# lhoangan/arap_flow

Hardware: AMD Instinct MI355X
Metric: ARAP solve+warp frames/sec at 854x480 mesh (higher is better)
Workload: dtype f32; 1 GPU; configs[1]: single 854x480 DAVIS-shaped frame, single-segment mask, fd=1; schedule 19/8/400; segments_per_frame=1, fd=1, parallelism=frames sharded, no collective, grid_vertices_per_frame=409920

## Files before the change

### arap_flow_amd/capi.py

```python
import ctypes as C
import os

_HERE = os.path.dirname(os.path.abspath(__file__))
LIB_PATH = os.environ.get("ARAPOPT_LIB") or os.path.join(_HERE, "lib", "libarapopt.so")


class Opt_InitializationParameters(C.Structure):
    _fields_ = [("doublePrecision", C.c_int), ("verbosityLevel", C.c_int),
                ("collectPerKernelTimingInfo", C.c_int), ("threadsPerBlock", C.c_int)]


class MeshStats(C.Structure):
    _fields_ = [("vertices", C.c_uint32), ("outside", C.c_uint32), ("triangles", C.c_uint32), ("folded", C.c_uint32),
                ("nonfinite", C.c_uint32), ("reserved", C.c_uint32), ("det_min", C.c_float), ("det_max", C.c_float),
                ("disp2_max", C.c_float)]


MESH_STATS_KEYS = tuple(k for k, _ in MeshStats._fields_ if k != "reserved")


_VP, _U, _I = C.c_void_p, C.c_uint, C.c_int
SYMBOLS = [
    ("Opt_NewState", _VP, [Opt_InitializationParameters]),
    ("Opt_ProblemDefine", _VP, [_VP, C.c_char_p, C.c_char_p]),
# ... 22 lines not shown
    ("ArapFlow_SolverSolve", _I, [_VP, _U, _U, _U, _U]),
    ("ArapFlow_SolverSolveAsync", _I, [_VP, _U, _U, _U, _U, _I, _I]),
    ("ArapFlow_SolverWait", _I, [_VP]),
    ("ArapFlow_SolverHostResults", _I, [_VP, _U, C.POINTER(_VP), C.POINTER(_VP), C.POINTER(_VP)]),
    ("ArapFlow_SolverWarp", _I, [_VP, _U]),
    ("ArapFlow_SolverGetResults", _I, [_VP, _U, _VP, _VP, _VP, _VP, _VP, C.POINTER(C.c_double)]),
    ("ArapFlow_SolverStats", _I, [_VP, C.POINTER(C.c_uint64), C.POINTER(C.c_uint64), C.POINTER(C.c_uint64)]),
    ("ArapFlow_SetResident", None, [_VP, _I]),
    ("ArapFlow_SetTile", _I, [_VP, _I, _I]),
    ("ArapFlow_SolverResidentLaunches", C.c_uint64, [_VP]),
    ("ArapFlow_PlanResidentLaunches", C.c_uint64, [_VP]),
    ("ArapFlow_SolverLaunchesFor", _I, [_VP, C.c_uint]),
    ("ArapFlow_ResidentDeal", _I, [C.POINTER(C.c_int), C.c_uint, C.POINTER(C.c_int), C.c_uint]),
    ("ArapFlow_ResidentTiles", _I, [_VP, _U, _U, _I, C.POINTER(C.c_int), _U, C.POINTER(C.c_int)]),
    ("ArapFlow_SolverResidentLayout", _I, [_VP, C.POINTER(C.c_int), C.POINTER(C.c_int)]),
    ("ArapFlow_SolverLeanStream", _I, [_VP]),
    ("ArapFlow_ResidentFailed", _I, [_VP]),
    ("ArapFlow_SolverStamps", _I, [_VP, _VP]),
    ("ArapFlow_SolverStampParts", _I, [_VP, _VP]),
    ("ArapFlow_WarpScratchBytes", C.c_uint64, [_U, _U]),
    ("ArapFlow_Warp", _I, [_VP, _U, _U, _VP, _VP, _VP, _VP, _VP, _VP]),
    ("ArapFlow_SolverSetOutputs", _I, [_VP, _I]),
    ("ArapFlow_SolverGetExtraResults", _I, [_VP, _U, _VP, _VP, _VP]),
    ("ArapFlow_SolverHostExtraResults", _I, [_VP, _U, C.POINTER(_VP), C.POINTER(_VP), C.POINTER(_VP)]),
    ("ArapFlow_WarpExScratchBytes", C.c_uint64, [_U, _U]),
    ("ArapFlow_WarpEx", _I, [_VP, _U, _U, _VP, _VP, _VP, _VP, _VP, _VP, _VP, _VP, _VP]),
    ("ArapFlow_SolverSetSnapshots", _I, [_VP, C.POINTER(C.c_uint), _U]),
    ("ArapFlow_SolverGetSnapshot", _I, [_VP, _U, _U, _VP, _VP, _VP, _VP]),
    ("ArapFlow_SolverHostSnapshot", _I, [_VP, _U, _U, C.POINTER(_VP), C.POINTER(_VP), C.POINTER(_VP), C.POINTER(_VP)]),
    ("ArapFlow_WarpStep", _I, [_VP, _U, _U, _VP, _VP, _VP, _VP, _VP, _VP, _VP]),
# ... 38 lines not shown
```

### arap_flow_amd/csrc/abi_solver.h

```cpp
#pragma once

namespace arap {
struct FrameExt {
    float2* bwd;
    uint8_t *occ_bwd, *occ;
    unsigned *cell, *rank;
    int4* bin;
};
struct MidDev {
    float2 *state, *flow, *step;
    uint8_t *rgb, *mask;
};
}

extern "C" int ArapFlow_SolverWait(ArapFlow_Solver* s);

enum { G_BASE, G_EXTRA, G_MID, G_DIAG, G_COUNT, MAX_PLANES = 5 };
enum { SEL_ALWAYS = 0, SEL_RGB = -1 , SEL_DEVICE = -2  };
struct Plane {
    size_t per_vertex, fixed;
    int sel;
    const void* (*dev)(const ArapFlow_Solver* s, unsigned slot, unsigned k);
};
static unsigned group_items(int g, unsigned state) { return g == G_MID ? state : state != 0; }
// ... 617 lines not shown
    build_resident_tiles(mask_red, (int)W, (int)H, aligned != 0, tiles, bx, nullptr);
    if (origins)
        for (size_t i = 0; i < tiles.size() && i < cap; ++i) origins[i] = tiles[i];
    if (bandx0)
        for (size_t i = 0; i < bx.size(); ++i) bandx0[i] = bx[i];
    return (int)tiles.size();
}
int ArapFlow_SolverResidentLayout(ArapFlow_Solver* s, int* launches_per_step, int* solves_in_flight)
{
    if (!s) return -1;
    const bool res = plan_resident_eligible(s->plan) && s->plan->res_sets > 0;
    if (launches_per_step) *launches_per_step = res ? s->plan->res_sets : 0;
    if (solves_in_flight) *solves_in_flight = res ? s->plan->res_inflight : 0;
    return 0;
}
int ArapFlow_ResidentFailed(Opt_State* state) { return state && state->resident_failed ? 1 : 0; }
int ArapFlow_SolverLeanStream(ArapFlow_Solver* s) { return s && plan_lean_stream(s->plan) ? 1 : 0; }

static int solver_stamp_table(ArapFlow_Solver* s, int table, uint64_t* out)
{
    if (!s || !s->plan->rd.stamps) return -1;
    HC(hipStreamSynchronize(s->st->stream));
    HC(hipMemcpy(out, s->plan->rd.stamps + table * RES_WGS * 16, RES_WGS * 16 * sizeof(unsigned long long), hipMemcpyDeviceToHost));
    return 0;
}
int ArapFlow_SolverStamps(ArapFlow_Solver* s, uint64_t* out) { return solver_stamp_table(s, 0, out); }
int ArapFlow_SolverStampParts(ArapFlow_Solver* s, uint64_t* out) { return solver_stamp_table(s, 1, out); }

}
```

### arap_flow_amd/csrc/arap_resident.h

```cpp
#pragma once
#include <type_traits>
#include "arap_device.h"

namespace arap {

constexpr int RES_WGS = 512;
constexpr int RES_MAX_GROUPS = 16;
constexpr int RES_THREADS = 256;
constexpr int RES_SLOTS = 9;
constexpr int RES_TILES_PER_WG = RES_SLOTS;
constexpr int RT_X = 32, RT_Y = 8;
constexpr int RES_ZX = 2 * RT_X + 2 * RT_Y;
constexpr int RES_ZG = 2 * RES_ZX;
constexpr int RES_MAX_L = 32000;
static_assert(RT_X * RT_Y == RES_THREADS && RT_Y == 2 * (RES_THREADS / 64), "one vertex per lane, two rows per wavefront");
constexpr int RES_MAX_HALO = RES_TILES_PER_WG * (2 * RT_X + 2 * RT_Y);
constexpr int RES_HALO_PER_THREAD = (RES_MAX_HALO + RES_THREADS - 1) / RES_THREADS;
constexpr int RES_MAX_TILES = RES_WGS * RES_TILES_PER_WG;
constexpr int LROW = RT_X + 2;
constexpr int LROWS = RT_Y + 2;
constexpr int LPLANE = LROW * LROWS;
constexpr int LTILE = 5 * LPLANE;
constexpr int RES_LDS_BYTES = RES_TILES_PER_WG * LTILE * 4
                              + ((RES_MAX_HALO * 8 + 15) / 16) * 16
// ... 3 lines not shown
#ifndef RES_HALO_REG_SLOTS
#define RES_HALO_REG_SLOTS 8
#endif
#ifndef RES_WREG_SLOTS
#define RES_WREG_SLOTS 7
#endif
#ifndef RES_WREG_8
#define RES_WREG_8 2
#endif
#ifndef RES_WREG_9
#define RES_WREG_9 2
#endif
#ifndef RES_WREG_FIT
#define RES_WREG_FIT 6
#endif
#ifndef RES_FIRST_LOOK
#define RES_FIRST_LOOK 5
#endif
#ifndef RES_FIRST_LOOK_2
#define RES_FIRST_LOOK_2 14
#endif
#ifndef RES_FIRST_LOOK_X
#define RES_FIRST_LOOK_X 20
#endif
#ifndef RES_OWN_LOCAL
#define RES_OWN_LOCAL 1
#endif
#ifndef RES_POLL_SLEEP
#define RES_POLL_SLEEP 1
#endif
constexpr unsigned RES_SPIN_LIMIT = 1u << 18;
#ifndef RES_GRAN_STRIDE
#define RES_GRAN_STRIDE 2
#endif
constexpr int RES_GS = RES_GRAN_STRIDE;
constexpr int RES_GRAN_UNITS = 2 * RES_WGS;
constexpr int RES_GRAN_L1 = 2 * RES_GRAN_UNITS * RES_GS;
constexpr int RES_GRAN2_STRIDE = 16;
constexpr int RES_GRAN2_GROUP = 2 * 8 * RES_GRAN2_STRIDE;
constexpr int RES_GRAN_X = RES_GRAN_L1 + 4 * RES_GRAN2_GROUP;
constexpr int RES_GRAN_PER_LAUNCH = RES_GRAN_X + RES_GRAN_L1;
#ifndef RES_FLAT_MAX_RUNS
#define RES_FLAT_MAX_RUNS 2
#endif

struct ResWg {
    int slot;
    int rank;
    int wgs;
    int gran;
};

struct ResDev {
    const int* tilelist;
    const int* ntiles;
    const int* tilepos;
    const int* bandx0;
    unsigned long long* zx;
    int rtX, rtY;
// ... 256 lines not shown
    v = wave_sum_l63_full(v);
    if (tb) { asm volatile("" :: "v"(v)); c1 = __builtin_amdgcn_s_memtime(); tb[0] += c1 - c0; c0 = c1; }
    const int wave = threadIdx.x >> 6, lane = threadIdx.x & 63;
    if (lane == 63) wsum[wave] = v;
    __syncthreads();
    double t = 0.0;
    if (wave == 0) {
        const double a = wsum[lane & 3], b = wsum[(lane & 3) ^ 1];
        if (tb) { asm volatile("s_waitcnt lgkmcnt(0)" ::: "memory"); c1 = __builtin_amdgcn_s_memtime(); tb[1] += c1 - c0; c0 = c1; }
        t = dpp_add_f64_full<0x112, 0xf>(a + b);
        if (tb) { asm volatile("" :: "v"(t)); c1 = __builtin_amdgcn_s_memtime(); tb[2] += c1 - c0; }
    }
    return t;
}

template <bool STAMPS, int NS>
__global__ __launch_bounds__(RES_THREADS, 2) void k_pcg_resident(PlanDev pd, ResDev rd, int L)
{
    static_assert(NS >= 1 && NS <= RES_SLOTS, "slots");
    unsigned long long tA = 0, tS1 = 0, tB = 0, tS2 = 0, tU = 0, t0 = 0, t1 = 0;
    unsigned long long tm[6] = {0, 0, 0, 0, 0, 0}, tbs = 0, tzr = 0;
    unsigned long long tbp[3] = {0, 0, 0}, tarr[2] = {0, 0};
#define RES_STAMP(acc) do { if (STAMPS) { t1 = __builtin_amdgcn_s_memrealtime(); acc += t1 - t0; t0 = t1; } } while (0)
    extern __shared__ __attribute__((aligned(16))) float lds[];
    const ResWg me = rd.wgmap[blockIdx.x];
    if (me.slot < 0) return;
    const int rank = me.rank;
    if (rd.force_fail) {
        if (threadIdx.x == 0) atomicExch(rd.err, 0xDEADFFFFu);
        return;
    }
    if (__hip_atomic_load(rd.err, __ATOMIC_RELAXED, __HIP_MEMORY_SCOPE_AGENT) != 0u) return;
    const int b = me.slot;
    const int wgs = me.wgs;
    const int W = pd.W, H = pd.H;
    const size_t gb = (size_t)b * pd.N;
    const int tid = threadIdx.x, lane = tid & 63, wave = tid >> 6;
    const int lx = lane & (RT_X - 1), ly = (wave << 1) | (lane >> 5);
    unsigned short* hlist = (unsigned short*)(lds + RES_TILES_PER_WG * LTILE);
    int2* tbase = (int2*)((char*)hlist + ((RES_MAX_HALO * 8 + 15) / 16) * 16);
    float* moLUT = (float*)(tbase + RES_TILES_PER_WG + 1);
    float* bcast = moLUT + 12;
    int* nhalo = (int*)(bcast + 4);
    double* wsum = (double*)(bcast + 6);
    unsigned* nbits = (unsigned*)(wsum + 10);
    unsigned* nremote = nbits + 16;
    float4* zst = (float4*)((char*)lds + RES_LDS_BYTES - RES_TILES_PER_WG * RES_ZX * 16);
    unsigned long long* gran_group = rd.gran + me.gran;
    unsigned long long* granx_group = rd.gran + RES_GRAN_X + me.gran;

    const int nt = rd.ntiles[b];
    const int tbase_n = nt / wgs, textra = nt - tbase_n * wgs;
    const int tp = tbase_n + (rank < textra ? 1 : 0);
    const int tfirst = rank * tbase_n + (rank < textra ? rank : textra);
    const int* tl = rd.tilelist + (size_t)b * RES_MAX_TILES;
    float wr2, wf2;
    {
        const Slot sl = pd.slots[b];
        wr2 = sl.wr * sl.wr;
        wf2 = sl.wf * sl.wf;
        if (tid < 10) {
            const int deg = tid % 5, fit = tid / 5;
            float dO = 0.f;
            for (int k = 0; k < deg; ++k) dO = dO + (sl.wr * sl.wr + sl.wr * sl.wr);
            if (fit) dO = fmaf(sl.wf, sl.wf, dO);
            moLUT[tid] = ginv(dO);
        }
        if (tid == 0) { *nhalo = 0; *nremote = 0u; }
        if (tid < 16) nbits[tid] = 0u;
    }

    float rx[NS], ry[NS], ra[NS];
    float dx_[NS], dy_[NS], da_[NS];
    float apx[NS], apy[NS], apa[NS];
    float ma_[NS], mo_[NS];
    unsigned fl[NS];
    int ibase[NS];
    constexpr int NWR = NS <= RES_WREG_SLOTS ? 4 : (NS == 8 ? RES_WREG_8 : RES_WREG_9);
    constexpr bool WREG = NWR > 0;
    float we[WREG ? NS : 1][5];
    const int loff = lx + W * ly;

    const int cell = (ly + 1) * LROW + (lx + 1);
#define TP2(T) ((float2*)(T))
#define TCS(T) ((float2*)(T) + LPLANE)
#define TPA(T) ((T) + 4 * LPLANE)

    int org_[NS];
#pragma unroll
    for (int j = 0; j < NS; ++j) org_[j] = j < tp ? tl[tfirst + j] : -1;
    unsigned long long* const zx_b = rd.zx + (size_t)b * RES_MAX_TILES * RES_ZG;
    for (int c = tid; c < tp * RES_ZG; c += RES_THREADS)
        __hip_atomic_store(zx_b + (size_t)tfirst * RES_ZG + c, 0ull, __ATOMIC_RELAXED, __HIP_MEMORY_SCOPE_AGENT);
// ... 55 lines not shown
        }
        fl[j] = qF[j];
        ibase[j] = __builtin_amdgcn_readfirstlane(x0 + W * y0);
        if (tid == 0) tbase[j] = make_int2(x0, y0);
    }
    float rho = read_scalar(pd.red + ((size_t)b * pd.nslots + 0) * NSHARD);
    __syncthreads();
#pragma unroll
    for (int j = 0; j < NS; ++j) {
        const unsigned f = fl[j];
        if (WREG) {
            if (NWR > 0) we[j][0] = keep_if<0>(f, wr2);
            if (NWR > 1) we[j][1] = keep_if<1>(f, wr2);
            if (NWR > 2) we[j][2] = keep_if<2>(f, wr2);
            if (NWR > 3) we[j][3] = keep_if<3>(f, wr2);
            if (NS <= RES_WREG_FIT) we[j][4] = keep_if<4>(f, wf2);
        }
        halo_append(ly == 0 && (f & F_E3), (unsigned short)(j * LPLANE + 0 * LROW + lx + 1), hlist, nhalo);
        halo_append(ly == RT_Y - 1 && (f & F_E2), (unsigned short)(j * LPLANE + (RT_Y + 1) * LROW + lx + 1), hlist, nhalo);
        halo_append(lx == 0 && (f & F_E1), (unsigned short)(j * LPLANE + (ly + 1) * LROW + 0), hlist, nhalo);
        halo_append(lx == RT_X - 1 && (f & F_E0), (unsigned short)(j * LPLANE + (ly + 1) * LROW + RT_X + 1), hlist, nhalo);
    }
    __syncthreads();
    const int nh = *nhalo;
    uint2* htab = (uint2*)hlist;
    constexpr bool HREG = NS <= RES_HALO_REG_SLOTS;
    uint2 hreg[RES_HALO_PER_THREAD];
    {
        uint2 e[RES_HALO_PER_THREAD];
#pragma unroll
        for (int u = 0; u < RES_HALO_PER_THREAD; ++u) {
// ... 36 lines not shown
            offP[n] = (unsigned)(cell + dn[n]) * 8u;
            offA[n] = (unsigned)(cell + dn[n]) * 4u;
            asm volatile("" : "+v"(offP[n]));
            asm volatile("" : "+v"(offA[n]));
        }
    }
    const int zent = border_entry(lx, ly);
    bool alive = true;
    float alpha_last = 0.f;
    asm volatile("s_waitcnt vmcnt(0)" ::: "memory");
    __syncthreads();
    bool fast = false, zfast = false;
    bool hier = false, subfast = false;
    bool hierx = false;
    unsigned long long* const gran2 =
        rd.gran + RES_GRAN_L1 + ((((int)(blockIdx.x & 7u) - (me.rank >> 6)) >> 1) & 3) * RES_GRAN2_GROUP;
    {
        const unsigned xcc = __builtin_amdgcn_s_getreg((3 << 11) | (0 << 6) | 20) & 15u;
        float dummy;
        const double mine = (double)xcc + 65536.0 * (double)(xcc * xcc);
        alive = group_sum(mine, 1u, gran_group, rank, wgs, bcast, rd.err, dummy, false, wsum + 8);
        const double tot = wsum[8];
        const double s2 = floor(tot / 65536.0), s1 = tot - 65536.0 * s2;
        fast = rd.allow_fast && ((double)wgs * s2 == s1 * s1);
        __syncthreads();
        hier = !fast && wgs > 64;
        hierx = hier && (((wgs + 63) >> 6) <= 2 || ((wgs + 63) >> 6) <= rd.flat_runs);
        if (!fast && rd.allow_fast && alive) {
            if (wave == 0) {
                const unsigned long long* buf = gran_group + (size_t)1 * wgs * RES_GS;
                bool remote = false, elsewhere = false;
                for (int m = lane; m < wgs; m += 64) {
                    const bool nb = ((nbits[(m >> 5) & 15] >> (m & 31)) & 1u) != 0u;
                    const bool same_run = hier && (m >> 6) == (rank >> 6);
                    if (nb || same_run) {
                        const unsigned long long lo = __hip_atomic_load(buf + RES_GS * m, __ATOMIC_RELAXED, __HIP_MEMORY_SCOPE_AGENT);
                        const unsigned long long hi = __hip_atomic_load(buf + RES_GS * m + 1, __ATOMIC_RELAXED, __HIP_MEMORY_SCOPE_AGENT);
                        const double val = __longlong_as_double((long long)((hi << 32) | (lo & 0xffffffffull)));
                        const double q2 = floor(val / 65536.0);
                        const bool other = (unsigned)(lo >> 32) != 1u || (unsigned)(hi >> 32) != 1u ||
                                           (unsigned)(val - 65536.0 * q2) != xcc;
                        remote = remote || (nb && other);
                        elsewhere = elsewhere || (same_run && other);
                    }
                }
                const unsigned any_remote = __any(remote) ? 1u : 0u, any_elsewhere = __any(elsewhere) ? 2u : 0u;
                if (lane == 0) *nremote = any_remote | any_elsewhere;
            }
            __syncthreads();
            zfast = (*nremote & 1u) == 0u;
            subfast = hier && (*nremote & 2u) == 0u;
        } else {
            zfast = fast;
        }
        __syncthreads();
    }
#ifndef RES_PRIO_HI
#define RES_PRIO_HI 2
#endif
#ifndef RES_PRIO_TAIL
#define RES_PRIO_TAIL 2
#endif
#define RES_PRIO(J) { if ((J) + RES_PRIO_TAIL >= NS) __builtin_amdgcn_s_setprio(0); else __builtin_amdgcn_s_setprio(RES_PRIO_HI); }
#define RES_PRIO_END() __builtin_amdgcn_s_setprio(0);
    if (STAMPS) t0 = __builtin_amdgcn_s_memrealtime();
    for (int l = 0; l < L && alive; ++l) {
// ... 52 lines not shown
                    const float2 t = fma2(make_float2(NQX, NQY), pa2, e);                              \
                    const float2 u = fma2(make_float2(NHX, NHY), make_float2(qA, qA), e + t);          \
                    axy = fma2(make_float2(w, w), u, axy);                                             \
                    aa = fmaf(-w, fmaf(QX, t.x, (QY) * t.y), aa);                                      \
                    (void)cn; (void)sn;                                                                \
                }
                RES_EDGE(0, 0,     -si,  ci,   -sn,  cn,    si, -ci)
                RES_EDGE(1, 1,      si, -ci,    sn, -cn,   -si,  ci)
                __builtin_amdgcn_sched_barrier(0);
                if (j + 1 < NS) RES_LOAD_B(j + 1)
                __builtin_amdgcn_sched_barrier(0);
                RES_EDGE(2, 2,     -ci, -si,   -cn, -sn,    ci,  si)
                RES_EDGE(3, 3,      ci,  si,    cn,  sn,   -ci, -si)
#undef RES_EDGE
                {
                    const float wf = (WREG && NS <= RES_WREG_FIT) ? we[WREG ? j : 0][4] : keep_if<4>(f, wf2);
                    axy = fma2(make_float2(wf, wf), pv, axy);
                }
                const float ax = axy.x, ay = axy.y;
                apx[j] = ax; apy[j] = ay; apa[j] = aa;
                acc += (double)dot3(pv.x, pv.y, pa_, ax, ay, aa);
            }
            __builtin_amdgcn_sched_barrier(0);
        }
#undef RES_LOAD_A
#undef RES_LOAD_B
        float sigma;
        RES_PRIO_END()
        RES_STAMP(tA);
        {
            const unsigned long long cb = STAMPS ? __builtin_amdgcn_s_memtime() : 0ull;
            const double bs = block_sum8(acc, wsum, STAMPS ? tbp : nullptr);
            if (STAMPS) tbs += __builtin_amdgcn_s_memtime() - cb;
            alive = hierx ? group_sum_x(block_sum_uniform(bs), 2u * l + 2u, gran_group, granx_group, rank, wgs, bcast, rd.err, sigma, subfast)
                  : hier  ? group_sum_h(block_sum_uniform(bs), 2u * l + 2u, gran_group, gran2, rank, wgs, bcast, rd.err, sigma, subfast)
                          : group_sum(bs, 2u * l + 2u, gran_group, rank, wgs, bcast, rd.err, sigma, fast, nullptr, rd.nowait != 0,
                                      STAMPS ? tm : nullptr, STAMPS ? tarr : nullptr);
        }
        asm volatile("" : "+v"(sigma));
        if (!alive) break;
        RES_STAMP(tS1);
        float alpha = 0.f;
        if (sigma > 0.f) alpha = rho / sigma;
        acc = 0.0;
        const unsigned ztag = 2u * l + 3u;
#pragma unroll
        for (int j = 0; j < NS; ++j) {
            RES_PRIO(j)
            unsigned f = fl[j];
            asm volatile("" : "+v"(f));
// ... 20 lines not shown
                const float2* const st2 = (const float2*)zst;
                const unsigned sh = (tid & 1) ? 16u : 0u;
                static_assert(((RES_THREADS - 64) & 1) == 0, "a thread keeps the parity of its granules");
                if (zfast) {
                    for (int g = tid - 64; g < tp * RES_ZG; g += RES_THREADS - 64) {
                        const float2 v = st2[g];
                        st_tagged(out + g, (ztag << 16) | ((__float_as_uint(v.y) >> sh) & 0xffffu), v.x, true);
                    }
                } else {
                    for (int g = tid - 64; g < tp * RES_ZG; g += RES_THREADS - 64) {
                        const float2 v = st2[g];
                        st_tagged(out + g, (ztag << 16) | ((__float_as_uint(v.y) >> sh) & 0xffffu), v.x, false);
                    }
                }
            }
            alive = hierx ? group_sum_x(block_sum_uniform(bs), 2u * l + 3u, gran_group, granx_group, rank, wgs, bcast, rd.err, rhoNew, subfast)
                  : hier  ? group_sum_h(block_sum_uniform(bs), 2u * l + 3u, gran_group, gran2, rank, wgs, bcast, rd.err, rhoNew, subfast)
                          : group_sum(bs, 2u * l + 3u, gran_group, rank, wgs, bcast, rd.err, rhoNew, fast, nullptr, rd.nowait != 0,
                                      STAMPS ? tm : nullptr, STAMPS ? tarr + 1 : nullptr);
        }
        unsigned long long hg[RES_HALO_PER_THREAD][2];
        unsigned hpk_[HREG ? 1 : RES_HALO_PER_THREAD];
#define RES_HPK(U) (HREG ? hreg[U].y : hpk_[HREG ? 0 : (U)])
#pragma unroll
        for (int u = 0; u < RES_HALO_PER_THREAD; ++u) {
            hg[u][0] = hg[u][1] = (unsigned long long)ztag << 48;
            if (tid + u * RES_THREADS < nh) {
                const unsigned gi = HREG ? hreg[u].x : htab[tid + u * RES_THREADS].x;
                const unsigned long long* q_ = (const unsigned long long*)((const char*)zx_b + (size_t)(gi * 8u));
#pragma unroll
                for (int c = 0; c < 2; ++c) hg[u][c] = __hip_atomic_load(q_ + c, __ATOMIC_RELAXED, __HIP_MEMORY_SCOPE_AGENT);
            }
// ... 163 lines not shown
```

### arap_flow_amd/csrc/host_plan.h

```cpp
#pragma once

static void hip_fatal(hipError_t e, const char* what, const char* file, int line)
{
    fprintf(stderr, "arapopt: HIP error %d (%s) in %s at %s:%d\n", (int)e, hipGetErrorString(e), what, file, line);
    exit((int)e ? (int)e : 1);
}
#define HC(call)                                                     \
    do {                                                             \
        hipError_t e_ = (call);                                      \
        if (e_ != hipSuccess) hip_fatal(e_, #call, __FILE__, __LINE__); \
    } while (0)

struct KernelTimer {
    struct Rec { std::string name; hipEvent_t a, b; };
    std::vector<Rec> recs;
    void clear()
    {
        for (auto& r : recs) { (void)hipEventDestroy(r.a); (void)hipEventDestroy(r.b); }
        recs.clear();
    }
    void report()
    {
        std::map<std::string, std::pair<int, double>> agg;
        for (auto& r : recs) {
// ... 23 lines not shown
}

struct Knobs {
    bool no_graph = false;
    int tile = -1;
    bool b8 = false;
    int stream_a = 0;
    bool no_resident = false;
    int force_res_fail = 0;
    bool no_xcd_fast = false;
    int flat_runs = RES_FLAT_MAX_RUNS;
    bool res_nowait = false;
    bool stamps = false;
    int res_groups = 0;
    int res_ns = 0;
};

static Knobs read_knobs()
{
    auto is = [](const char* name, char c) { const char* v = getenv(name); return v && v[0] == c; };
    auto num = [](const char* name, int absent) { const char* v = getenv(name); return v ? atoi(v) : absent; };
    Knobs k;
    k.no_graph = is("ARAPOPT_NO_GRAPH", '1');
    if (const char* tv = getenv("ARAPOPT_TILE")) {
        int tx = -1, ty = -1;
        if (sscanf(tv, "%dx%d", &tx, &ty) == 2) k.tile = tile_shape_index(tx, ty);
    }
    k.b8 = is("ARAPOPT_B8", '1');
    k.stream_a = num("ARAPOPT_STREAM_A", 0);
    k.no_resident = is("ARAPOPT_NO_RESIDENT", '1');
    k.force_res_fail = is("ARAPOPT_FORCE_RES_FAIL", '1') ? 1 : (is("ARAPOPT_FORCE_RES_FAIL", '2') ? 2 : 0);
    k.no_xcd_fast = is("ARAPOPT_NO_XCD_FAST", '1');
    k.flat_runs = num("ARAPOPT_FLAT_RUNS", RES_FLAT_MAX_RUNS);
    k.res_nowait = is("ARAPOPT_RES_NOWAIT", '1');
    k.stamps = is("ARAPOPT_STAMPS", '1');
    k.res_groups = std::max(0, num("ARAPOPT_RES_GROUPS", 0));
    k.res_ns = std::max(0, num("ARAPOPT_RES_NS", 0));
    return k;
}

struct Opt_State {
    int verbosity = 0;
    int timing = 0;
    int device = 0;
    hipStream_t stream = nullptr;
    hipStream_t cap = nullptr;
    hipStream_t own_stream = nullptr;
    hipEvent_t t0 = nullptr, t1 = nullptr;
    KernelTimer ktimer;
    bool use_graph = true;
    bool use_resident = true;
    bool resident_failed = false;
// ... 14 lines not shown
          q_tolerance = 1e-4f, function_tolerance = 1e-6f, trust_region_radius = 1e4f,
          radius_decrease_factor = 2.0f, min_lm_diagonal = 1e-6f, max_lm_diagonal = 1e32f;
    int nIterations = 10, lIterations = 10;
    int nIter = 0;
};

enum { GN_STEP_ALL = 0, GN_STEP_PREP = 1, GN_STEP_FUSED = 2 };
enum PhaseA { PA_NONE = 0, PA_DIRECT, PA_LDS_16x16, PA_LDS_32x8, PA_LDS_64x4, PA_LDS_32x16, PA_LDS_64x8,
              PA_MARCH, PA_MARCH2, PA_GRID };
enum PhaseB { PB_NONE = 0, PB_B, PB_B4, PB_B4_LEAN, PB_B4_R };
struct StepRecipe {
    bool resident = false;
    int part = GN_STEP_ALL;
    int L = -1, nb = 0, nsteps = 0;
    std::vector<int> res_ns;
    bool stamped = false;
    int list_blocks = 0;
    int a_kern = PA_NONE, b_kern = PB_NONE;
    dim3 a_grid{0, 0, 0}, a_block{0, 0, 0};
    int a_arg[3] = {0, 0, 0};
    int lag = -1;
};
static bool same_recipe(const StepRecipe& a, const StepRecipe& b)
{
    auto same3 = [](dim3 x, dim3 y) { return x.x == y.x && x.y == y.y && x.z == y.z; };
    return a.resident == b.resident && a.part == b.part && a.L == b.L && a.nb == b.nb && a.nsteps == b.nsteps &&
           a.res_ns == b.res_ns && a.stamped == b.stamped && a.list_blocks == b.list_blocks && a.a_kern == b.a_kern &&
           a.b_kern == b.b_kern && same3(a.a_grid, b.a_grid) && same3(a.a_block, b.a_block) &&
           std::equal(a.a_arg, a.a_arg + 3, b.a_arg) && a.lag == b.lag;
}

struct Opt_Plan {
    Opt_State* st = nullptr;
    int W = 0, H = 0, N = 0, batch = 1;
    PlanDev pd{};
    SolverParameters sp;
    std::vector<Slot> hslots;
    std::vector<Slot> uploaded;
    void* block = nullptr;
    int lcap = 0;
    int ccap = 0;
    int nb = 1;
// ... 11 lines not shown
    std::vector<std::vector<int>> h_tiles;
    std::vector<uint8_t> h_tiles_valid;
    std::vector<std::vector<int>> h_tilepos, h_bandx0;
    uint8_t* d_resact = nullptr;
    int* d_t64list = nullptr;
    int* d_t64n = nullptr;
    std::vector<std::vector<int>> h_t64;
    std::vector<int> h_t64n;
    int res_tiles_all = 0;
    bool hole_pending = false;
    ResWg* d_wgmap = nullptr;
    ResWg* pin_wgmap = nullptr;
    std::vector<ResWg> h_wgmap;
    int res_sets = 0;
    std::vector<int> res_ns;
    int knob_res_groups = 0, knob_res_ns = 0;
    int res_inflight = 0;
    unsigned res_launches = 0;
    bool opt_res_ok = false;
    bool prep_done = false;
    Slot opt_res_slot{};
    int* d_notgrid = nullptr;
    int kind = 0;
    void* lm_block = nullptr;
    float2* prevO = nullptr;
    float* prevA = nullptr;
    int lm_lcap = 0;
    float lm_radius = 0.f, lm_decrease = 0.f;
    double lm_prev_cost = 0.0;
    bool lm_done = false;

// ... 127 lines not shown
```

### arap_flow_amd/csrc/host_resident.h

```cpp
#pragma once

typedef void (*ResidentKernel)(PlanDev, ResDev, int);
template <bool STAMPS, int... NS>
static const void* resident_kernel_of(int ns, std::integer_sequence<int, NS...>)
{
    static const ResidentKernel table[] = {k_pcg_resident<STAMPS, NS + 1>...};
    return (const void*)table[ns - 1];
}
static const void* resident_kernel(bool stamps, int ns)
{
    if (ns < 1) ns = 1;
    if (ns > RES_SLOTS) ns = RES_SLOTS;
    return stamps ? resident_kernel_of<true>(ns, std::make_integer_sequence<int, RES_SLOTS>())
                  : resident_kernel_of<false>(ns, std::make_integer_sequence<int, RES_SLOTS>());
}

static void plan_enable_resident(Opt_Plan* p)
{
    Opt_State* st = p->st;
    const Knobs knobs = read_knobs();
    p->knob_res_groups = knobs.res_groups;
    p->knob_res_ns = knobs.res_ns;
    if (knobs.no_resident) return;
    hipDeviceProp_t prop;
    HC(hipGetDeviceProperties(&prop, st->device));
    if (prop.multiProcessorCount * 2 < RES_WGS) return;
    for (int ns = 1; ns <= RES_SLOTS; ++ns) {
        if (hipFuncSetAttribute(resident_kernel(false, ns), hipFuncAttributeMaxDynamicSharedMemorySize, RES_LDS_BYTES) !=
            hipSuccess) { (void)hipGetLastError(); return; }
        int occ = 0;
        if (hipOccupancyMaxActiveBlocksPerMultiprocessor(&occ, resident_kernel(false, ns), RES_THREADS, RES_LDS_BYTES) !=
                hipSuccess || occ < 2) {
            (void)hipGetLastError();
            return;
        }
    }
    const size_t B = (size_t)p->batch;
    const size_t sz_map = align_up(B * RES_WGS * sizeof(ResWg), 256);
    p->rd.rtX = (p->W + RT_X - 1) / RT_X;
    p->rd.rtY = (p->H + RT_Y - 1) / RT_Y;
    {
        const size_t nz = B * RES_MAX_TILES * RES_ZG * sizeof(unsigned long long);
        HC(hipMalloc((void**)&p->rd.zx, nz));
        HC(hipMemsetAsync(p->rd.zx, 0, nz, st->stream));
    }
    HC(hipHostMalloc((void**)&p->pin_wgmap, sz_map, hipHostMallocDefault));
    p->res_block = device_block(st, true, [&](Carver& part) {
        part(p->rd.gran, B * RES_GRAN_PER_LAUNCH * 8);
        part(p->rd.tilelist, B * RES_MAX_TILES * sizeof(int));
        part(p->rd.ntiles, B * sizeof(int));
        part(p->rd.err, sizeof(unsigned));
        part(p->d_wgmap, sz_map);
        part(p->rd.tilepos, B * p->rd.rtX * p->rd.rtY * sizeof(int));
        part(p->rd.bandx0, B * p->rd.rtY * sizeof(int));
        part(p->d_resact, (size_t)p->rd.rtX * p->rd.rtY);
    });
    p->pd.res_err = p->rd.err;
    p->rd.stamps = nullptr;
    p->rd.force_fail = knobs.force_res_fail == 1 ? 1 : 0;
    p->hole_pending = knobs.force_res_fail == 2;
    p->rd.allow_fast = knobs.no_xcd_fast ? 0 : 1;
    p->rd.flat_runs = knobs.flat_runs;
    p->rd.nowait = knobs.res_nowait ? 1 : 0;
    if (knobs.stamps) {
        for (int ns = 1; ns <= RES_SLOTS; ++ns)
            HC(hipFuncSetAttribute(resident_kernel(true, ns), hipFuncAttributeMaxDynamicSharedMemorySize, RES_LDS_BYTES));
        HC(hipMalloc(&p->rd.stamps, 2 * RES_WGS * 16 * sizeof(unsigned long long)));
        HC(hipMemset(p->rd.stamps, 0, 2 * RES_WGS * 16 * sizeof(unsigned long long)));
    }
    p->res_capable = true;
}

static void build_resident_tiles(const uint8_t* mask_red, int W, int H, bool aligned, std::vector<int>& tiles,
                                 std::vector<int>& bandx0, uint64_t* nactive)
{
    const int rtY = (H + RT_Y - 1) / RT_Y;
    tiles.clear();
    bandx0.assign(rtY, 0);
    std::vector<uint8_t> col(W);
    uint64_t na = 0;
    for (int band = 0; band < rtY; ++band) {
// ... 250 lines not shown
                    if (kind[b] == WIDE || bin_of[b] != (int)k) continue;
                    take_gran(b);
                    const int r0 = kind[b] == MEDIUM ? XW : 0;
                    for (int r = 0; r < part_w[b]; ++r, ++j)
                        map[(size_t)set * RES_WGS + (size_t)j * 8 + x] = ResWg{b, r0 + r, wgs_of[b], gran_of[b]};
                }
            }
            inflight = count > inflight ? count : inflight;
        }
    }
    if (map_out) map_out->swap(map);
    if (inflight_out) *inflight_out = inflight;
    return nsets;
}

static bool plan_resident_pack(Opt_Plan* p)
{
    std::vector<ResWg> map;
    const int nsets = resident_deal(p->h_ntiles.data(), p->nb, p->knob_res_groups, &map, &p->res_inflight);
    std::vector<int> ns(nsets, 1);
    for (size_t i = 0; i < map.size(); ++i)
        if (map[i].slot >= 0) {
            const int t = (p->h_ntiles[map[i].slot] + map[i].wgs - 1) / map[i].wgs;
            int& m = ns[i / RES_WGS];
            m = t > m ? t : m;
        }
    if (p->knob_res_ns > 0)
        for (int& m : ns) m = std::max(m, std::min(p->knob_res_ns, (int)RES_SLOTS));
    const bool same = nsets == p->res_sets && ns == p->res_ns && map.size() == p->h_wgmap.size() &&
                      memcmp(map.data(), p->h_wgmap.data(), map.size() * sizeof(ResWg)) == 0;
    if (same) return false;
    p->h_wgmap.swap(map);
    p->res_ns.swap(ns);
    p->res_sets = nsets;
    return true;
}

static void plan_upload_wgmap(Opt_Plan* p)
{
    Opt_State* st = p->st;
    if (p->hole_pending) {
        std::vector<ResWg> holed = p->h_wgmap;
        for (ResWg& w : holed)
            if (w.slot >= 0 && w.wgs > 1 && w.rank == w.wgs - 1) { w = ResWg{-1, 0, 0, 0}; break; }
        HC(hipStreamSynchronize(st->stream));
        HC(hipMemcpy(p->d_wgmap, holed.data(), holed.size() * sizeof(ResWg), hipMemcpyHostToDevice));
        p->hole_pending = false;
    } else {
// ... 34 lines not shown
```

### arap_flow_amd/csrc/host_step.h

```cpp
#pragma once

static bool plan_active_tiles_majority(const Opt_Plan* p)
{
    long act = 0;
    for (int b = 0; b < p->nb; ++b) act += p->h_ntiles[b];
    const long all = (long)((p->W + RT_X - 1) / RT_X) * ((p->H + RT_Y - 1) / RT_Y);
    return 2 * act >= (long)p->nb * all;
}

static bool plan_lean_stream(const Opt_Plan* p)
{
    return p->res_frames_any && p->grid_u && !p->pd.lm && p->st->tile < 0 && (p->N & 3) == 0 && !p->st->force_b8 &&
           p->st->stream_a == 0 && plan_active_tiles_majority(p);
}

static int plan_list_blocks(const Opt_Plan* p)
{
    int maxn = 1;
    for (int k = 0; k < p->nb; ++k) maxn = std::max(maxn, p->h_t64n[k]);
    return std::min((maxn + 63) / 64 * 64, p->pd.tilesX * p->pd.tilesY);
}

constexpr int MARCH_ROWS = 5, MARCH2_ROWS = 7;

static StepRecipe plan_step_recipe(Opt_Plan* p, int nsteps)
{
    const Opt_State* st = p->st;
    StepRecipe r;
    r.resident = plan_resident_eligible(p);
    r.L = p->sp.lIterations;
    r.nb = p->nb;
    r.nsteps = nsteps;
    if (r.resident) {
        if (plan_resident_pack(p)) plan_upload_wgmap(p);
        r.res_ns = p->res_ns;
        r.stamped = p->rd.stamps != nullptr;
        if (p->res_frames && st->verbosity == 0) r.part = GN_STEP_FUSED;
        if (p->res_frames && p->d_t64list != nullptr) r.list_blocks = plan_list_blocks(p);
        return r;
    }
    const bool lean = plan_lean_stream(p);
    int v = st->tile;
    if (v < 0 && p->grid_u && !p->pd.lm) {
        if (st->stream_a == 1) {
            constexpr int TX = 64, TY = 8;
            const int tX = (p->W + TX - 1) / TX, tY = (p->H + TY - 1) / TY, ch = (tX * tY + 7) / 8;
            r.a_kern = PA_GRID;
            r.a_grid = dim3((unsigned)(p->nb * 8 * ch));
            r.a_block = dim3(TX, TY, 1);
            r.a_arg[0] = tX; r.a_arg[1] = tY; r.a_arg[2] = ch;
// ... 70 lines not shown
    if (r.list_blocks > 0) {
        pd.t64list = pdl.t64list = p->d_t64list;
        pd.t64n = pdl.t64n = p->d_t64n;
        gl = dim3((unsigned)r.list_blocks, 1, (unsigned)r.nb);
    }
    if (part != GN_STEP_FUSED) LAUNCH(p, s, "GNPrep", k_gn_prep, gl, b, 0, pd);
    if (part == GN_STEP_PREP) return;
    if (part == GN_STEP_FUSED) LAUNCH(p, s, "PCGInit1", k_gn_init_resf, gl, b, 0, pd);
    else LAUNCH(p, s, "PCGInit1", k_gn_init, gl, b, 0, pdl);
    if (r.resident) {
        ResDev rd = p->rd;
        rd.fuse_update = part == GN_STEP_FUSED ? 1 : 0;
        for (size_t set = 0; set < r.res_ns.size(); ++set) {
            rd.wgmap = p->d_wgmap + set * RES_WGS;
            rd.gran = p->rd.gran + gran_per_launch * set;
            const ResidentKernel kern = (ResidentKernel)resident_kernel(r.stamped, r.res_ns[set]);
            if (r.stamped)
                hipLaunchKernelGGL(kern, dim3(RES_WGS), dim3(RES_THREADS), RES_LDS_BYTES, s, p->pd, rd, L);
            else
                LAUNCH(p, s, "PCGResident", kern, dim3(RES_WGS), dim3(RES_THREADS), RES_LDS_BYTES, p->pd, rd, L);
        }
    } else {
        for (int l = 0; l < L; ++l) {
            launch_pcg_a(p, s, r, l);
            launch_pcg_b(p, s, r, l);
        }
    }
    if (part != GN_STEP_FUSED) LAUNCH(p, s, "PCGLinearUpdate", k_gn_update, gl, b, 0, pdl, r.lag);
}

static void plan_gn_step(Opt_Plan* p, int nsteps = 1)
// ... 88 lines not shown
```

### arap_flow_amd/opt.py

```python
import ctypes as C
import math

import numpy as np
import torch

from . import capi

BUILTIN_PLAN = b"builtin:arap"


def _dev_ptr(t):
    assert t.is_cuda and t.is_contiguous()
    return C.c_void_p(t.data_ptr())


def _host_ptr(a):
    return a.ctypes.data_as(C.c_void_p) if a is not None else None


def _view(ptr, ctype, shape):
    if not ptr.value:
        return None
    return np.ctypeslib.as_array(C.cast(ptr, C.POINTER(ctype)), shape=(int(np.prod(shape)),)).reshape(shape)

# ... 374 lines not shown
            obwd = np.empty((H, W), np.uint8) if self.outputs & capi.OUT_BACKWARD else None
            occ = np.empty((H, W), np.uint8) if self.outputs & capi.OUT_OCCLUSION else None
            if self.lib.ArapFlow_SolverGetExtraResults(self.h, slot, p(bwd), p(obwd), p(occ)) != 0:
                return out
            if bwd is not None:
                out.update(backward_flow=bwd, occlusion_bwd=obwd)
            if occ is not None:
                out.update(occlusion=occ)
        return out

    def stats(self):
        a, b, c = C.c_uint64(), C.c_uint64(), C.c_uint64()
        self.lib.ArapFlow_SolverStats(self.h, C.byref(a), C.byref(b), C.byref(c))
        ls, fl = C.c_int(0), C.c_int(0)
        self.lib.ArapFlow_SolverResidentLayout(self.h, C.byref(ls), C.byref(fl))
        return dict(pcg_iterations_per_frame=a.value, active_vertices=b.value, grid_vertices=c.value,
                    resident_launches=int(self.lib.ArapFlow_SolverResidentLaunches(self.h)),
                    resident_launches_per_step=ls.value, resident_solves_in_flight=fl.value,
                    lean_stream=bool(self.lib.ArapFlow_SolverLeanStream(self.h)))

    def close(self):
        if self.h:
            self.lib.ArapFlow_SolverFree(self.h)
            self.h = None


def _warp_call(state, name, dims, inputs, outputs, scratch=None, bad_args=True, lead=()):
    lib = state.lib
    up = lambda a, dt: None if a is None else torch.from_numpy(np.ascontiguousarray(a, dt)).cuda()
    new = lambda shape, dt: None if shape is None else torch.empty(*shape, dtype=dt, device="cuda")
    lead = [up(*a) if isinstance(a, tuple) else a for a in lead]
    args = [[up(x, dt) for x in a] if isinstance(a, list) else up(a, dt) for a, dt in inputs]
    outs = {k: [new(q, dt) for q in shape] if isinstance(shape, list) else new(shape, dt) for k, shape, dt in outputs}
# ... 159 lines not shown
```

### include/arap_opt.h

```cpp
#ifndef ARAP_OPT_H
#define ARAP_OPT_H

#include <stdint.h>

#ifdef __cplusplus
extern "C" {
#endif


typedef struct Opt_State Opt_State;
typedef struct Opt_Plan Opt_Plan;
typedef struct Opt_Problem Opt_Problem;

struct Opt_InitializationParameters {
    int doublePrecision;
    int verbosityLevel;
    int collectPerKernelTimingInfo;
    int threadsPerBlock;
};
typedef struct Opt_InitializationParameters Opt_InitializationParameters;

Opt_State* Opt_NewState(Opt_InitializationParameters params);

Opt_Problem* Opt_ProblemDefine(Opt_State* state, const char* filename, const char* solverkind);
// ... 65 lines not shown
int ArapFlow_SolverHostSnapshot(ArapFlow_Solver* s, unsigned slot, unsigned k, const float** flow, const uint8_t** rgb,
                                const uint8_t** mask, const float** step);

int ArapFlow_SolverWarp(ArapFlow_Solver* s, unsigned nframes);

int ArapFlow_SolverGetResults(ArapFlow_Solver* s, unsigned slot, float* flow, uint8_t* warped_rgb,
                              uint8_t* warped_mask, float* offset, float* angle, double* final_cost);

int ArapFlow_SolverStats(ArapFlow_Solver* s, uint64_t* pcg_iterations_per_frame, uint64_t* active_vertices,
                         uint64_t* grid_vertices);

void ArapFlow_SetResident(Opt_State* state, int on);
int ArapFlow_SetTile(Opt_State* state, int tile_x, int tile_y);
uint64_t ArapFlow_SolverResidentLaunches(ArapFlow_Solver* s);
int ArapFlow_SolverResidentLayout(ArapFlow_Solver* s, int* launches_per_step, int* solves_in_flight);
int ArapFlow_SolverLaunchesFor(ArapFlow_Solver* s, unsigned nframes);
int ArapFlow_ResidentDeal(const int* active_tiles, unsigned nsolves, int* table, unsigned table_launches);
int ArapFlow_ResidentTiles(const uint8_t* mask_red, unsigned W, unsigned H, int aligned, int* origins, unsigned cap,
                           int* bandx0);
uint64_t ArapFlow_PlanResidentLaunches(Opt_Plan* plan);
int ArapFlow_ResidentFailed(Opt_State* state);
int ArapFlow_SolverLeanStream(ArapFlow_Solver* s);
int ArapFlow_SolverStamps(ArapFlow_Solver* s, uint64_t* out);
int ArapFlow_SolverStampParts(ArapFlow_Solver* s, uint64_t* out);

uint64_t ArapFlow_WarpScratchBytes(unsigned W, unsigned H);
int ArapFlow_Warp(Opt_State* state, unsigned W, unsigned H, const void* rgb, const void* mask_red,
                  const void* flow, void* out_rgb, void* out_mask, void* scratch);

uint64_t ArapFlow_WarpExScratchBytes(unsigned W, unsigned H);
// ... 47 lines not shown
```

Before: 29.76 frames/s.

## Add flat-group-sum resident kernel variant that reuses freed registers for weights

Adds a SUMS template flavour to the persistent PCG kernel. When every solve in a launch uses at most RES_WGS/8 workgroups, the host selects a FLAT variant that compiles out the hierarchical group-sum paths. The registers this frees go to caching more per-edge weights (the fit weight up to 7 slots and different NWR for 8/9 slots). This is meant to cut register pressure and global weight reloads in the inner matvec. It doubles the number of kernel instantiations, and the occupancy check now covers both flavours, so a failure in either disables resident mode entirely.

Result: faster. 30.70 frames/s (median of 6 runs) (+3.2%).

```diff
diff --git a/arap_flow_amd/capi.py b/arap_flow_amd/capi.py
--- a/arap_flow_amd/capi.py
+++ b/arap_flow_amd/capi.py
@@ -60,6 +60,7 @@
     ("ArapFlow_ResidentDeal", _I, [C.POINTER(C.c_int), C.c_uint, C.POINTER(C.c_int), C.c_uint]),
     ("ArapFlow_ResidentTiles", _I, [_VP, _U, _U, _I, C.POINTER(C.c_int), _U, C.POINTER(C.c_int)]),
     ("ArapFlow_SolverResidentLayout", _I, [_VP, C.POINTER(C.c_int), C.POINTER(C.c_int)]),
+    ("ArapFlow_SolverResidentSums", _I, [_VP, C.POINTER(C.c_int), C.c_uint]),
     ("ArapFlow_SolverLeanStream", _I, [_VP]),
     ("ArapFlow_ResidentFailed", _I, [_VP]),
     ("ArapFlow_SolverStamps", _I, [_VP, _VP]),
diff --git a/arap_flow_amd/csrc/abi_solver.h b/arap_flow_amd/csrc/abi_solver.h
--- a/arap_flow_amd/csrc/abi_solver.h
+++ b/arap_flow_amd/csrc/abi_solver.h
@@ -655,6 +655,14 @@
     if (solves_in_flight) *solves_in_flight = res ? s->plan->res_inflight : 0;
     return 0;
 }
+int ArapFlow_SolverResidentSums(ArapFlow_Solver* s, int* sums, unsigned cap)
+{
+    if (!s) return -1;
+    const Opt_Plan* p = s->plan;
+    if (!plan_resident_eligible(p) || p->res_sets <= 0) return 0;
+    for (int k = 0; k < p->res_sets && sums && (unsigned)k < cap; ++k) sums[k] = p->res_sums[k];
+    return p->res_sets;
+}
 int ArapFlow_ResidentFailed(Opt_State* state) { return state && state->resident_failed ? 1 : 0; }
 int ArapFlow_SolverLeanStream(ArapFlow_Solver* s) { return s && plan_lean_stream(s->plan) ? 1 : 0; }
 
diff --git a/arap_flow_amd/csrc/arap_resident.h b/arap_flow_amd/csrc/arap_resident.h
--- a/arap_flow_amd/csrc/arap_resident.h
+++ b/arap_flow_amd/csrc/arap_resident.h
@@ -41,6 +41,15 @@
 #ifndef RES_WREG_FIT
 #define RES_WREG_FIT 6
 #endif
+#ifndef RES_WREG_FIT_FLAT
+#define RES_WREG_FIT_FLAT 7
+#endif
+#ifndef RES_WREG_8_FLAT
+#define RES_WREG_8_FLAT 3
+#endif
+#ifndef RES_WREG_9_FLAT
+#define RES_WREG_9_FLAT RES_WREG_9
+#endif
 #ifndef RES_FIRST_LOOK
 #define RES_FIRST_LOOK 5
 #endif
@@ -70,6 +79,8 @@
 #ifndef RES_FLAT_MAX_RUNS
 #define RES_FLAT_MAX_RUNS 2
 #endif
+
+constexpr int RES_SUMS_ANY = 0, RES_SUMS_FLAT = 1, RES_SUMS_COUNT = 2;
 
 struct ResWg {
     int slot;
@@ -356,10 +367,14 @@
     return t;
 }
 
-template <bool STAMPS, int NS>
+template <bool STAMPS, int NS, int SUMS>
 __global__ __launch_bounds__(RES_THREADS, 2) void k_pcg_resident(PlanDev pd, ResDev rd, int L)
 {
     static_assert(NS >= 1 && NS <= RES_SLOTS, "slots");
+    static_assert(SUMS == RES_SUMS_ANY || SUMS == RES_SUMS_FLAT, "group-sum flavour");
+    constexpr bool FLAT = SUMS == RES_SUMS_FLAT;
+    constexpr bool SPEND = FLAT && !STAMPS;
+    constexpr int WFIT = SPEND ? RES_WREG_FIT_FLAT : RES_WREG_FIT;
     unsigned long long tA = 0, tS1 = 0, tB = 0, tS2 = 0, tU = 0, t0 = 0, t1 = 0;
     unsigned long long tm[6] = {0, 0, 0, 0, 0, 0}, tbs = 0, tzr = 0;
     unsigned long long tbp[3] = {0, 0, 0}, tarr[2] = {0, 0};
@@ -389,7 +404,7 @@
     unsigned* nremote = nbits + 16;
     float4* zst = (float4*)((char*)lds + RES_LDS_BYTES - RES_TILES_PER_WG * RES_ZX * 16);
     unsigned long long* gran_group = rd.gran + me.gran;
-    unsigned long long* granx_group = rd.gran + RES_GRAN_X + me.gran;
+    unsigned long long* granx_group = FLAT ? nullptr : rd.gran + RES_GRAN_X + me.gran;
 
     const int nt = rd.ntiles[b];
     const int tbase_n = nt / wgs, textra = nt - tbase_n * wgs;
@@ -418,7 +433,8 @@
     float ma_[NS], mo_[NS];
     unsigned fl[NS];
     int ibase[NS];
-    constexpr int NWR = NS <= RES_WREG_SLOTS ? 4 : (NS == 8 ? RES_WREG_8 : RES_WREG_9);
+    constexpr int NWR = NS <= RES_WREG_SLOTS ? 4 : (NS == 8 ? (SPEND ? RES_WREG_8_FLAT : RES_WREG_8)
+                                                            : (SPEND ? RES_WREG_9_FLAT : RES_WREG_9));
     constexpr bool WREG = NWR > 0;
     float we[WREG ? NS : 1][5];
     const int loff = lx + W * ly;
@@ -504,7 +520,7 @@
             if (NWR > 1) we[j][1] = keep_if<1>(f, wr2);
             if (NWR > 2) we[j][2] = keep_if<2>(f, wr2);
             if (NWR > 3) we[j][3] = keep_if<3>(f, wr2);
-            if (NS <= RES_WREG_FIT) we[j][4] = keep_if<4>(f, wf2);
+            if (NS <= WFIT) we[j][4] = keep_if<4>(f, wf2);
         }
         halo_append(ly == 0 && (f & F_E3), (unsigned short)(j * LPLANE + 0 * LROW + lx + 1), hlist, nhalo);
         halo_append(ly == RT_Y - 1 && (f & F_E2), (unsigned short)(j * LPLANE + (RT_Y + 1) * LROW + lx + 1), hlist, nhalo);
@@ -571,7 +587,7 @@
     bool hier = false, subfast = false;
     bool hierx = false;
     unsigned long long* const gran2 =
-        rd.gran + RES_GRAN_L1 + ((((int)(blockIdx.x & 7u) - (me.rank >> 6)) >> 1) & 3) * RES_GRAN2_GROUP;
+        FLAT ? nullptr : rd.gran + RES_GRAN_L1 + ((((int)(blockIdx.x & 7u) - (me.rank >> 6)) >> 1) & 3) * RES_GRAN2_GROUP;
     {
         const unsigned xcc = __builtin_amdgcn_s_getreg((3 << 11) | (0 << 6) | 20) & 15u;
         float dummy;
@@ -581,7 +597,7 @@
         const double s2 = floor(tot / 65536.0), s1 = tot - 65536.0 * s2;
         fast = rd.allow_fast && ((double)wgs * s2 == s1 * s1);
         __syncthreads();
-        hier = !fast && wgs > 64;
+        hier = !FLAT && !fast && wgs > 64;
         hierx = hier && (((wgs + 63) >> 6) <= 2 || ((wgs + 63) >> 6) <= rd.flat_runs);
         if (!fast && rd.allow_fast && alive) {
             if (wave == 0) {
@@ -606,7 +622,7 @@
             }
             __syncthreads();
             zfast = (*nremote & 1u) == 0u;
-            subfast = hier && (*nremote & 2u) == 0u;
+            subfast = !FLAT && hier && (*nremote & 2u) == 0u;
         } else {
             zfast = fast;
         }
@@ -689,7 +705,7 @@
                 RES_EDGE(3, 3,      ci,  si,    cn,  sn,   -ci, -si)
 #undef RES_EDGE
                 {
-                    const float wf = (WREG && NS <= RES_WREG_FIT) ? we[WREG ? j : 0][4] : keep_if<4>(f, wf2);
+                    const float wf = (WREG && NS <= WFIT) ? we[WREG ? j : 0][4] : keep_if<4>(f, wf2);
                     axy = fma2(make_float2(wf, wf), pv, axy);
                 }
                 const float ax = axy.x, ay = axy.y;
@@ -707,8 +723,8 @@
             const unsigned long long cb = STAMPS ? __builtin_amdgcn_s_memtime() : 0ull;
             const double bs = block_sum8(acc, wsum, STAMPS ? tbp : nullptr);
             if (STAMPS) tbs += __builtin_amdgcn_s_memtime() - cb;
-            alive = hierx ? group_sum_x(block_sum_uniform(bs), 2u * l + 2u, gran_group, granx_group, rank, wgs, bcast, rd.err, sigma, subfast)
-                  : hier  ? group_sum_h(block_sum_uniform(bs), 2u * l + 2u, gran_group, gran2, rank, wgs, bcast, rd.err, sigma, subfast)
+            alive = (!FLAT && hierx) ? group_sum_x(block_sum_uniform(bs), 2u * l + 2u, gran_group, granx_group, rank, wgs, bcast, rd.err, sigma, subfast)
+                  : (!FLAT && hier)  ? group_sum_h(block_sum_uniform(bs), 2u * l + 2u, gran_group, gran2, rank, wgs, bcast, rd.err, sigma, subfast)
                           : group_sum(bs, 2u * l + 2u, gran_group, rank, wgs, bcast, rd.err, sigma, fast, nullptr, rd.nowait != 0,
                                       STAMPS ? tm : nullptr, STAMPS ? tarr : nullptr);
         }
@@ -759,8 +775,8 @@
                     }
                 }
             }
-            alive = hierx ? group_sum_x(block_sum_uniform(bs), 2u * l + 3u, gran_group, granx_group, rank, wgs, bcast, rd.err, rhoNew, subfast)
-                  : hier  ? group_sum_h(block_sum_uniform(bs), 2u * l + 3u, gran_group, gran2, rank, wgs, bcast, rd.err, rhoNew, subfast)
+            alive = (!FLAT && hierx) ? group_sum_x(block_sum_uniform(bs), 2u * l + 3u, gran_group, granx_group, rank, wgs, bcast, rd.err, rhoNew, subfast)
+                  : (!FLAT && hier)  ? group_sum_h(block_sum_uniform(bs), 2u * l + 3u, gran_group, gran2, rank, wgs, bcast, rd.err, rhoNew, subfast)
                           : group_sum(bs, 2u * l + 3u, gran_group, rank, wgs, bcast, rd.err, rhoNew, fast, nullptr, rd.nowait != 0,
                                       STAMPS ? tm : nullptr, STAMPS ? tarr + 1 : nullptr);
         }
diff --git a/arap_flow_amd/csrc/host_plan.h b/arap_flow_amd/csrc/host_plan.h
--- a/arap_flow_amd/csrc/host_plan.h
+++ b/arap_flow_amd/csrc/host_plan.h
@@ -61,6 +61,7 @@
     bool stamps = false;
     int res_groups = 0;
     int res_ns = 0;
+    bool res_sums_any = false;
 };
 
 static Knobs read_knobs()
@@ -83,6 +84,7 @@
     k.stamps = is("ARAPOPT_STAMPS", '1');
     k.res_groups = std::max(0, num("ARAPOPT_RES_GROUPS", 0));
     k.res_ns = std::max(0, num("ARAPOPT_RES_NS", 0));
+    k.res_sums_any = is("ARAPOPT_RES_SUMS", 'a');
     return k;
 }
 
@@ -127,6 +129,7 @@
     int part = GN_STEP_ALL;
     int L = -1, nb = 0, nsteps = 0;
     std::vector<int> res_ns;
+    std::vector<int> res_sums;
     bool stamped = false;
     int list_blocks = 0;
     int a_kern = PA_NONE, b_kern = PB_NONE;
@@ -138,7 +141,7 @@
 {
     auto same3 = [](dim3 x, dim3 y) { return x.x == y.x && x.y == y.y && x.z == y.z; };
     return a.resident == b.resident && a.part == b.part && a.L == b.L && a.nb == b.nb && a.nsteps == b.nsteps &&
-           a.res_ns == b.res_ns && a.stamped == b.stamped && a.list_blocks == b.list_blocks && a.a_kern == b.a_kern &&
+           a.res_ns == b.res_ns && a.res_sums == b.res_sums && a.stamped == b.stamped && a.list_blocks == b.list_blocks && a.a_kern == b.a_kern &&
            a.b_kern == b.b_kern && same3(a.a_grid, b.a_grid) && same3(a.a_block, b.a_block) &&
            std::equal(a.a_arg, a.a_arg + 3, b.a_arg) && a.lag == b.lag;
 }
@@ -180,7 +183,9 @@
     std::vector<ResWg> h_wgmap;
     int res_sets = 0;
     std::vector<int> res_ns;
+    std::vector<int> res_sums;
     int knob_res_groups = 0, knob_res_ns = 0;
+    bool knob_res_sums_any = false;
     int res_inflight = 0;
     unsigned res_launches = 0;
     bool opt_res_ok = false;
diff --git a/arap_flow_amd/csrc/host_resident.h b/arap_flow_amd/csrc/host_resident.h
--- a/arap_flow_amd/csrc/host_resident.h
+++ b/arap_flow_amd/csrc/host_resident.h
@@ -1,19 +1,22 @@
 #pragma once
 
 typedef void (*ResidentKernel)(PlanDev, ResDev, int);
-template <bool STAMPS, int... NS>
+template <bool STAMPS, int SUMS, int... NS>
 static const void* resident_kernel_of(int ns, std::integer_sequence<int, NS...>)
 {
-    static const ResidentKernel table[] = {k_pcg_resident<STAMPS, NS + 1>...};
+    static const ResidentKernel table[] = {k_pcg_resident<STAMPS, NS + 1, SUMS>...};
     return (const void*)table[ns - 1];
 }
-static const void* resident_kernel(bool stamps, int ns)
+static const void* resident_kernel(bool stamps, int ns, int sums)
 {
     if (ns < 1) ns = 1;
     if (ns > RES_SLOTS) ns = RES_SLOTS;
-    return stamps ? resident_kernel_of<true>(ns, std::make_integer_sequence<int, RES_SLOTS>())
-                  : resident_kernel_of<false>(ns, std::make_integer_sequence<int, RES_SLOTS>());
-}
+    const auto slots = std::make_integer_sequence<int, RES_SLOTS>();
+    if (sums == RES_SUMS_FLAT)
+        return stamps ? resident_kernel_of<true, RES_SUMS_FLAT>(ns, slots) : resident_kernel_of<false, RES_SUMS_FLAT>(ns, slots);
+    return stamps ? resident_kernel_of<true, RES_SUMS_ANY>(ns, slots) : resident_kernel_of<false, RES_SUMS_ANY>(ns, slots);
+}
+static const char* resident_sums_name(int sums) { return sums == RES_SUMS_FLAT ? "flat" : "any"; }
 
 static void plan_enable_resident(Opt_Plan* p)
 {
@@ -21,20 +24,24 @@
     const Knobs knobs = read_knobs();
     p->knob_res_groups = knobs.res_groups;
     p->knob_res_ns = knobs.res_ns;
+    p->knob_res_sums_any = knobs.res_sums_any;
     if (knobs.no_resident) return;
     hipDeviceProp_t prop;
     HC(hipGetDeviceProperties(&prop, st->device));
     if (prop.multiProcessorCount * 2 < RES_WGS) return;
-    for (int ns = 1; ns <= RES_SLOTS; ++ns) {
-        if (hipFuncSetAttribute(resident_kernel(false, ns), hipFuncAttributeMaxDynamicSharedMemorySize, RES_LDS_BYTES) !=
-            hipSuccess) { (void)hipGetLastError(); return; }
-        int occ = 0;
-        if (hipOccupancyMaxActiveBlocksPerMultiprocessor(&occ, resident_kernel(false, ns), RES_THREADS, RES_LDS_BYTES) !=
-                hipSuccess || occ < 2) {
-            (void)hipGetLastError();
-            return;
-        }
-    }
+    for (int sums = 0; sums < RES_SUMS_COUNT; ++sums)
+        for (int ns = 1; ns <= RES_SLOTS; ++ns) {
+            const void* kern = resident_kernel(false, ns, sums);
+            if (hipFuncSetAttribute(kern, hipFuncAttributeMaxDynamicSharedMemorySize, RES_LDS_BYTES) != hipSuccess) {
+                (void)hipGetLastError();
+                return;
+            }
+            int occ = 0;
+            if (hipOccupancyMaxActiveBlocksPerMultiprocessor(&occ, kern, RES_THREADS, RES_LDS_BYTES) != hipSuccess || occ < 2) {
+                (void)hipGetLastError();
+                return;
+            }
+        }
     const size_t B = (size_t)p->batch;
     const size_t sz_map = align_up(B * RES_WGS * sizeof(ResWg), 256);
     p->rd.rtX = (p->W + RT_X - 1) / RT_X;
@@ -63,8 +70,9 @@
     p->rd.flat_runs = knobs.flat_runs;
     p->rd.nowait = knobs.res_nowait ? 1 : 0;
     if (knobs.stamps) {
-        for (int ns = 1; ns <= RES_SLOTS; ++ns)
-            HC(hipFuncSetAttribute(resident_kernel(true, ns), hipFuncAttributeMaxDynamicSharedMemorySize, RES_LDS_BYTES));
+        for (int sums = 0; sums < RES_SUMS_COUNT; ++sums)
+            for (int ns = 1; ns <= RES_SLOTS; ++ns)
+                HC(hipFuncSetAttribute(resident_kernel(true, ns, sums), hipFuncAttributeMaxDynamicSharedMemorySize, RES_LDS_BYTES));
         HC(hipMalloc(&p->rd.stamps, 2 * RES_WGS * 16 * sizeof(unsigned long long)));
         HC(hipMemset(p->rd.stamps, 0, 2 * RES_WGS * 16 * sizeof(unsigned long long)));
     }
@@ -345,6 +353,14 @@
     return nsets;
 }
 
+static int resident_launch_sums(const ResWg* map, bool force_any)
+{
+    if (force_any) return RES_SUMS_ANY;
+    for (int i = 0; i < RES_WGS; ++i)
+        if (map[i].slot >= 0 && map[i].wgs > RES_WGS / 8) return RES_SUMS_ANY;
+    return RES_SUMS_FLAT;
+}
+
 static bool plan_resident_pack(Opt_Plan* p)
 {
     std::vector<ResWg> map;
@@ -358,11 +374,15 @@
         }
     if (p->knob_res_ns > 0)
         for (int& m : ns) m = std::max(m, std::min(p->knob_res_ns, (int)RES_SLOTS));
-    const bool same = nsets == p->res_sets && ns == p->res_ns && map.size() == p->h_wgmap.size() &&
+    std::vector<int> sums(nsets, RES_SUMS_ANY);
+    for (int set = 0; set < nsets; ++set)
+        sums[set] = resident_launch_sums(map.data() + (size_t)set * RES_WGS, p->knob_res_sums_any);
+    const bool same = nsets == p->res_sets && ns == p->res_ns && sums == p->res_sums && map.size() == p->h_wgmap.size() &&
                       memcmp(map.data(), p->h_wgmap.data(), map.size() * sizeof(ResWg)) == 0;
     if (same) return false;
     p->h_wgmap.swap(map);
     p->res_ns.swap(ns);
+    p->res_sums.swap(sums);
     p->res_sets = nsets;
     return true;
 }
diff --git a/arap_flow_amd/csrc/host_step.h b/arap_flow_amd/csrc/host_step.h
--- a/arap_flow_amd/csrc/host_step.h
+++ b/arap_flow_amd/csrc/host_step.h
@@ -34,6 +34,7 @@
     if (r.resident) {
         if (plan_resident_pack(p)) plan_upload_wgmap(p);
         r.res_ns = p->res_ns;
+        r.res_sums = p->res_sums;
         r.stamped = p->rd.stamps != nullptr;
         if (p->res_frames && st->verbosity == 0) r.part = GN_STEP_FUSED;
         if (p->res_frames && p->d_t64list != nullptr) r.list_blocks = plan_list_blocks(p);
@@ -134,7 +135,7 @@
         for (size_t set = 0; set < r.res_ns.size(); ++set) {
             rd.wgmap = p->d_wgmap + set * RES_WGS;
             rd.gran = p->rd.gran + gran_per_launch * set;
-            const ResidentKernel kern = (ResidentKernel)resident_kernel(r.stamped, r.res_ns[set]);
+            const ResidentKernel kern = (ResidentKernel)resident_kernel(r.stamped, r.res_ns[set], r.res_sums[set]);
             if (r.stamped)
                 hipLaunchKernelGGL(kern, dim3(RES_WGS), dim3(RES_THREADS), RES_LDS_BYTES, s, p->pd, rd, L);
             else
diff --git a/arap_flow_amd/opt.py b/arap_flow_amd/opt.py
--- a/arap_flow_amd/opt.py
+++ b/arap_flow_amd/opt.py
@@ -412,9 +412,13 @@
         self.lib.ArapFlow_SolverStats(self.h, C.byref(a), C.byref(b), C.byref(c))
         ls, fl = C.c_int(0), C.c_int(0)
         self.lib.ArapFlow_SolverResidentLayout(self.h, C.byref(ls), C.byref(fl))
+        sums = (C.c_int * 64)()
+        n = max(0, min(64, self.lib.ArapFlow_SolverResidentSums(self.h, sums, 64)))
+        names = ["flat" if sums[k] == 1 else "any" for k in range(n)]
         return dict(pcg_iterations_per_frame=a.value, active_vertices=b.value, grid_vertices=c.value,
                     resident_launches=int(self.lib.ArapFlow_SolverResidentLaunches(self.h)),
                     resident_launches_per_step=ls.value, resident_solves_in_flight=fl.value,
+                    resident_sums=names[0] if len(set(names)) == 1 else ",".join(names),
                     lean_stream=bool(self.lib.ArapFlow_SolverLeanStream(self.h)))
 
     def close(self):
diff --git a/include/arap_opt.h b/include/arap_opt.h
--- a/include/arap_opt.h
+++ b/include/arap_opt.h
@@ -103,6 +103,7 @@
 int ArapFlow_SetTile(Opt_State* state, int tile_x, int tile_y);
 uint64_t ArapFlow_SolverResidentLaunches(ArapFlow_Solver* s);
 int ArapFlow_SolverResidentLayout(ArapFlow_Solver* s, int* launches_per_step, int* solves_in_flight);
+int ArapFlow_SolverResidentSums(ArapFlow_Solver* s, int* sums, unsigned cap);
 int ArapFlow_SolverLaunchesFor(ArapFlow_Solver* s, unsigned nframes);
 int ArapFlow_ResidentDeal(const int* active_tiles, unsigned nsolves, int* table, unsigned table_launches);
 int ArapFlow_ResidentTiles(const uint8_t* mask_red, unsigned W, unsigned H, int aligned, int* origins, unsigned cap,
```
